# shravan-d/SculptMate

Measured on AMD Instinct MI355X. Metric: meshes/sec + ms/image, TripoSR 256^3 grid, at 1/2/4/8 MI355X, higher is better.
Workload: dtype fp32-equivalent (bf16 3-limb split, 24 bits, fp32 accumulate) density MLP / f32 tables, SiLU, marching cubes / bf16 transformer [filtered grid: an fp16 one-product pass decides the SIGN away from the level, every value marching cubes reads carries the three-limb value: mesh bit-identical to the full

## Files before the change

### include/sculpt_hip.h

```cpp
#ifndef SCULPT_HIP_H
#define SCULPT_HIP_H

#include <stddef.h>
#include <stdint.h>

#ifdef __cplusplus
extern "C" {
#endif

#define SCULPT_ABI_VERSION 4

typedef void *sculpt_stream_t;

int sculpt_version(void);
const char *sculpt_source_digest(void);
const char *sculpt_last_error(void);
int sculpt_device_count(void);
int sculpt_stream_create_cu_mask(int first_cu, int n_cus, sculpt_stream_t *stream_out);
int sculpt_stream_destroy(sculpt_stream_t stream);

size_t sculpt_mlp_packed_bytes(int in_channels, int n_hidden_64);
int sculpt_mlp_pack(const float *const *W_host, const float *const *b_host, int n_layers,
                    const int *dims_host, void *packed_host, size_t packed_bytes);

// ... 201 lines not shown
                         sculpt_stream_t stream);

int sculpt_resize_aa_bilinear(const float *in_hwc, int Hin, int Win, int C, float *tmp, float *out_hwc, int Hout,
                              int Wout, sculpt_stream_t stream);

int sculpt_resample_lanczos_ksize(int in_size, int out_size);
int sculpt_resample_lanczos_coeffs(int in_size, int out_size, int ksize, int32_t *bounds_host, int32_t *kk_host);
int sculpt_resample_u8(const uint8_t *in_hwc, int Hin, int Win, int C, const int32_t *bounds_x, const int32_t *kk_x, int ksize_x,
                       const int32_t *bounds_y, const int32_t *kk_y, int ksize_y, uint8_t *tmp, uint8_t *out_hwc, int Hout, int Wout,
                       sculpt_stream_t stream);
int sculpt_u2net_input(const uint8_t *img_hwc, int H, int W, int C, const double *mean3_host, const double *std3_host, int32_t *ws,
                       float *out_chw, sculpt_stream_t stream);
int sculpt_u2net_mask(const float *d0, int64_t n, uint32_t *ws, uint8_t *mask, sculpt_stream_t stream);
int sculpt_cutout_bbox(const uint8_t *img_hwc, const uint8_t *mask, int H, int W, int C, int32_t *ws, int32_t *bbox_host,
                       sculpt_stream_t stream);
int sculpt_cutout_frame(const uint8_t *img_hwc, const uint8_t *mask, int H, int W, int C, int y0, int x0, int h, int w, int top,
                        int left, int S, int grey, uint8_t *out, sculpt_stream_t stream);
int sculpt_u8_to_unit_f32(const uint8_t *in, int64_t n, float *out, sculpt_stream_t stream);

int sculpt_vit_patchify(const float *image_hwc, int S, int P, const float *mean3_host, const float *std3_host,
                        uint16_t *patches, float *patches_f32 , int ld, sculpt_stream_t stream);
int sculpt_vit_assemble(const float *patch_out, const float *cls, const float *pos, float *tokens,
                        int n_patches, int hidden, sculpt_stream_t stream);

int sculpt_upsample_scatter(const float *g, int ldg, const float *bias, float *planes, int S, int Co,
                            sculpt_stream_t stream);

size_t sculpt_bake_workspace_bytes(int res);
int sculpt_bake_rasterize(const float *uv, size_t nv, const int *idx, size_t nf, int res, void *workspace,
                          float *out, sculpt_stream_t stream);
int sculpt_bake_interpolate(const float *attr, size_t nv, const int *idx, size_t nf, const float *rast, int res,
                            float *out, sculpt_stream_t stream);
void rasterize_cpu(const float *uv, size_t nv, const int *idx, size_t nf, long long res, float *out);
void interpolate_cpu(const float *attr, size_t nv, const int *idx, size_t nf, const float *rast, long long res,
                     float *out);

int sculpt_im2col3x3(const void *in, int n_planes, int S, int C, int elem_bytes, void *out, sculpt_stream_t stream);
int sculpt_pixel_shuffle(const float *g, int ldg, float *planes, int n_planes, int S, int Co, int r,
                         sculpt_stream_t stream);

int sculpt_normalize_rows3(const float *x, int64_t n, float eps, float *y, sculpt_stream_t stream);

int sculpt_bake_material(const float *rast, int res, const float *color, const float *perturb_normal, const float *nrm,
                         const float *tng, float *albedo, float *bump, sculpt_stream_t stream);

int sculpt_uv_cell_atlas(const float *v_pos, const void *faces, int faces_i64, int64_t nf, int cols, int rows, float padding,
// ... 146 lines not shown
```

### sculptmate_amd/_lib.py

```python
import ctypes
import os

import torch

_HERE = os.path.dirname(os.path.abspath(__file__))
SO_PATH = os.path.join(_HERE, "libsculpt_hip.so")


class SculptError(RuntimeError):
    def __init__(self, msg, code=1):
        super().__init__(msg)
        self.code = code


if not os.path.exists(SO_PATH):
    raise ImportError(
        "sculptmate_amd: %s is missing -- build it with `python -m sculptmate_amd.build` "
        "(or __graft_entry__.build()); there is no CPU fallback." % SO_PATH)


def _load_matching_library():
    from . import build as _build

    if os.environ.get("SCULPT_ALLOW_STALE_LIB") == "1":
# ... 80 lines not shown
    "sculpt_maxpool2x2_ceil": (_i, [_vp, _i, _i, _i, _i, _vp, _i, _vp]),
    "sculpt_upsample_bilinear_bf16": (_i, [_vp, _i, _i, _i, _i, _vp, _i, _i, _i, _vp]),
    "sculpt_upsample_bilinear_f32": (_i, [_vp, _i, _i, _i, _vp, _i, _i, _vp]),
    "sculpt_add_bf16": (_i, [_vp, _i, _vp, _i, _vp, _i, _i64, _i, _vp]),
    "sculpt_fuse_sigmoid": (_i, [_vp, _i, _i64, _vp, _f, _vp, _vp]),
    "sculpt_gemm_f32": (_i, [_vp, _i, _vp, _i, _vp, _vp, _i, _vp, _i, _vp, _i, _i, _i, _i, _i, _i, _f, _i, _vp]),
    "sculpt_attention_f32_l3": (_i, [_vp, _i, _vp, _i, _vp, _i, _vp, _i, _i, _i, _i, _f, _vp]),
    "sculpt_limbs_bytes": (_sz, [_i, _i, _i]),
    "sculpt_attention_f32_l3_batched": (_i, [_vp, _i, _i64, _vp, _i, _i64, _vp, _i, _i64, _vp, _i, _i64, _vp, _i, _i, _i, _i, _i, _i, _i, _i, _f, _i, _vp]),
    "sculpt_layernorm_limbs": (_i, [_vp, _i, _vp, _vp, _f, _vp, _i, _vp, _i, _i, _i, _vp]),
    "sculpt_attention_f32_l3_limbs": (_i, [_vp, _i, _vp, _i, _vp, _i, _vp, _i, _i, _i, _i, _i, _i, _f, _i, _vp]),
    "sculpt_limbs_split": (_i, [_vp, _i, _i, _i, _f, _i, _vp, _vp]),
    "sculpt_gemm_l3p": (_i, [_vp, _vp, _i, _f, _vp, _vp, _i, _vp, _i, _vp, _i, _i, _vp, _i, _i, _i, _i, _i, _vp]),
    "sculpt_gemm_f32_ex": (_i, [_vp, _i, _vp, _i, _vp, _vp, _i, _vp, _i, _vp, _i, _i, _i, _i, _i, _i, _f, _i, _i, _i, _i64, _i64, _i64, _vp]),
    "sculpt_softmax_rows_f32": (_i, [_vp, _i, _i, _i, _i, _vp]),
    "sculpt_attention_bf16": (_i, [_vp, _i, _vp, _i, _vp, _i, _vp, _i, _i, _i, _i, _f, _vp]),
    "sculpt_attention_bf16_prescaled": (_i, [_vp, _i, _vp, _i, _vp, _i, _vp, _i, _i, _i, _i, _vp]),
    "sculpt_attention_bf16_batched": (_i, [_vp, _i, _i64, _vp, _i, _i64, _vp, _i, _i64, _vp, _i, _i64, _i, _i, _i, _i, _i, _f, _vp]),
    "sculpt_layernorm": (_i, [_vp, _vp, _i, _vp, _vp, _f, _vp, _i, _vp, _i, _i, _vp]),
    "sculpt_groupnorm_tokens": (_i, [_vp, _i, _i, _i, _vp, _vp, _f, _vp, _vp, _vp, _vp]),
    "sculpt_transpose_add": (_i, [_vp, _vp, _vp, _i, _i, _vp]),
    "sculpt_vit_patchify": (_i, [_vp, _i, _i, _vp, _vp, _vp, _vp, _i, _vp]),
    "sculpt_vit_assemble": (_i, [_vp, _vp, _vp, _vp, _i, _i, _vp]),
    "sculpt_upsample_scatter": (_i, [_vp, _i, _vp, _vp, _i, _i, _vp]),
    "sculpt_cast_bf16": (_i, [_vp, _vp, _i64, _vp]),
    "sculpt_dilate_fill": (_i, [_vp, _vp, _i, _i, _i, _vp, _vp, _vp]),
    "sculpt_vertex_accumulate_workspace_bytes": (_sz, [_sz]),
    "sculpt_vertex_normals": (_i, [_vp, _sz, _vp, _i, _sz, _vp, _vp, _vp]),
    "sculpt_vertex_tangents": (_i, [_vp, _vp, _vp, _sz, _vp, _i, _sz, _vp, _vp, _vp]),
    "sculpt_resize_aa_bilinear": (_i, [_vp, _i, _i, _i, _vp, _vp, _i, _i, _vp]),
    "sculpt_resample_lanczos_ksize": (_i, [_i, _i]),
    "sculpt_resample_lanczos_coeffs": (_i, [_i, _i, _i, _vp, _vp]),
    "sculpt_resample_u8": (_i, [_vp, _i, _i, _i, _vp, _vp, _i, _vp, _vp, _i, _vp, _vp, _i, _i, _vp]),
    "sculpt_u2net_input": (_i, [_vp, _i, _i, _i, _vp, _vp, _vp, _vp, _vp]),
    "sculpt_u2net_mask": (_i, [_vp, _i64, _vp, _vp, _vp]),
    "sculpt_cutout_bbox": (_i, [_vp, _vp, _i, _i, _i, _vp, _vp, _vp]),
    "sculpt_cutout_frame": (_i, [_vp, _vp, _i, _i, _i, _i, _i, _i, _i, _i, _i, _i, _i, _vp, _vp]),
    "sculpt_u8_to_unit_f32": (_i, [_vp, _i64, _vp, _vp]),
    "sculpt_bake_workspace_bytes": (_sz, [_i]),
    "sculpt_bake_rasterize": (_i, [_vp, _sz, _vp, _sz, _i, _vp, _vp, _vp]),
    "sculpt_bake_interpolate": (_i, [_vp, _sz, _vp, _sz, _vp, _i, _vp, _vp]),
    "sculpt_im2col3x3": (_i, [_vp, _i, _i, _i, _i, _vp, _vp]),
    "sculpt_pixel_shuffle": (_i, [_vp, _i, _vp, _i, _i, _i, _i, _vp]),
    "sculpt_uv_stats_words": (_sz, []),
    "sculpt_uv_moments_workspace_bytes": (_sz, []),
    "sculpt_uv_moments": (_i, [_vp, _sz, _vp, _vp, _vp]),
# ... 116 lines not shown
```

### sculptmate_amd/csrc/norms.hip

```cpp
#include "common.h"
#include "limbs.h"

namespace sculpt {

__device__ __forceinline__ float wave_sum(float v) {
#pragma unroll
    for (int d = 32; d >= 1; d >>= 1) v += __shfl_xor(v, d, 64);
    return v;
}

template <bool IN_BF16>
__global__ __launch_bounds__(256) void layernorm_kernel(const float *__restrict__ xf, const uint16_t *__restrict__ xb,
                                                        int ldx, const float *__restrict__ gamma,
                                                        const float *__restrict__ beta, float eps,
                                                        uint16_t *__restrict__ y, int ldy, float *__restrict__ yf,
                                                        int rows, int cols, unsigned char *__restrict__ y_lt = nullptr, int lt_fmt = 0) {
    const int lane = threadIdx.x & 63;
    const int row = blockIdx.x * 4 + (threadIdx.x >> 6);
    if (row >= rows) return;
    constexpr int MAXV = 8;
    float v[MAXV][4];
    const int nv = cols / 256;
    float s = 0.f;
#pragma unroll
// ... 158 lines not shown
    }
}

__global__ __launch_bounds__(256) void upsample_scatter_kernel(const float *__restrict__ g, int ldg,
                                                               const float *__restrict__ bias, float *__restrict__ planes,
                                                               int S, int Co) {
    const int S2 = 2 * S;
    const long total = 3L * Co * S2 * S2;
    for (long i = (long)blockIdx.x * 256 + threadIdx.x; i < total; i += (long)gridDim.x * 256) {
        const int X = (int)(i % S2), Y = (int)((i / S2) % S2);
        const int co = (int)((i / ((long)S2 * S2)) % Co), pl = (int)(i / ((long)S2 * S2 * Co));
        const int w = X >> 1, dx = X & 1, hh = Y >> 1, dy = Y & 1;
        const long tok = (long)pl * S * S + (long)hh * S + w;
        planes[i] = g[tok * ldg + co * 4 + dy * 2 + dx] + bias[co];
    }
}

__global__ __launch_bounds__(256) void cast_bf16_kernel(const float *__restrict__ x, uint16_t *__restrict__ y, long n) {
    for (long i = (long)blockIdx.x * 256 + threadIdx.x; i < n; i += (long)gridDim.x * 256) y[i] = f32_to_bf16(x[i]);
}

static inline int grid_for(long n) { return (int)std::min<long>((n + 255) / 256, 2048); }

__global__ __launch_bounds__(256) void row_slice_stats_kernel(const float *__restrict__ x, int ldx, int rows, int slots,
                                                              float *__restrict__ stats, int stats_ld,
                                                              uint16_t *__restrict__ xb, int ldb) {
    const long t = (long)blockIdx.x * 256 + threadIdx.x;
    if (t >= (long)rows * slots) return;
    const int slot = (int)(t / rows), row = (int)(t % rows);
    const float4 *src = reinterpret_cast<const float4 *>(x + (long)row * ldx + slot * 64);
    float4 v[16];
    float s = 0.f;
#pragma unroll
    for (int i = 0; i < 16; ++i) { v[i] = src[i]; s += (v[i].x + v[i].y) + (v[i].z + v[i].w); }
    const float mean = s * (1.0f / 64.0f);
    float m2 = 0.f;
#pragma unroll
    for (int i = 0; i < 16; ++i) {
        const float a = v[i].x - mean, b = v[i].y - mean, c = v[i].z - mean, d = v[i].w - mean;
        m2 = fmaf(a, a, m2); m2 = fmaf(b, b, m2); m2 = fmaf(c, c, m2); m2 = fmaf(d, d, m2);
    }
    reinterpret_cast<float2 *>(stats)[(long)slot * stats_ld + row] = make_float2(mean, m2);
    if (xb) {
        uint2 *dst = reinterpret_cast<uint2 *>(xb + (long)row * ldb + slot * 64);
#pragma unroll
        for (int i = 0; i < 16; ++i) {
            uint2 pk;
            pk.x = pack_bf16x2(v[i].x, v[i].y);
            pk.y = pack_bf16x2(v[i].z, v[i].w);
            dst[i] = pk;
        }
    }
}

}

using namespace sculpt;

extern "C" {

int sculpt_row_slice_stats(const float *x, int ldx, int rows, int cols, float *stats, int stats_ld, uint16_t *x_bf16, int ldb,
                           sculpt_stream_t stream) {
    SC_REQUIRE(x && stats && stats_ld >= rows, "row_slice_stats: null argument or stats_ld < rows");
    SC_REQUIRE(cols >= 64 && cols % 64 == 0 && ldx % 4 == 0 && (!x_bf16 || ldb % 4 == 0), "row_slice_stats: cols=%d must be a multiple of 64", cols);
    if (rows <= 0) return 0;
    const int slots = cols / 64;
    hipLaunchKernelGGL(row_slice_stats_kernel, dim3(cdiv((long)rows * slots, 256)), dim3(256), 0, as_stream(stream), x, ldx, rows,
                       slots, stats, stats_ld, x_bf16, ldb);
    SC_LAUNCH_CHECK();
    return 0;
}

int sculpt_layernorm(const float *x_f32, const uint16_t *x_bf16, int ldx, const float *gamma, const float *beta,
                     float eps, uint16_t *y, int ldy, float *y_f32, int rows, int cols, sculpt_stream_t stream) {
    SC_REQUIRE((x_f32 != nullptr) != (x_bf16 != nullptr), "layernorm: give exactly one of x_f32 / x_bf16");
// ... 51 lines not shown

int sculpt_vit_patchify(const float *image_hwc, int S, int P, const float *mean3_host, const float *std3_host,
                        uint16_t *patches, float *patches_f32, int ld, sculpt_stream_t stream) {
    SC_REQUIRE(image_hwc && mean3_host && std3_host && (patches || patches_f32), "vit_patchify: null argument");
    SC_REQUIRE(P > 0 && S >= P, "vit_patchify: bad S=%d P=%d", S, P);
    if (ld <= 0) ld = 3 * P * P;
    SC_REQUIRE(ld >= 3 * P * P, "vit_patchify: ld=%d < 3*P*P", ld);
    const long total = (long)(S / P) * (S / P) * ld;
    hipLaunchKernelGGL(patchify_kernel, dim3(grid_for(total)), dim3(256), 0, as_stream(stream), image_hwc, S, P, ld,
                       mean3_host[0], mean3_host[1], mean3_host[2], std3_host[0], std3_host[1], std3_host[2], patches, patches_f32);
    SC_LAUNCH_CHECK();
    return 0;
}

int sculpt_vit_assemble(const float *patch_out, const float *cls, const float *pos, float *tokens, int n_patches,
                        int hidden, sculpt_stream_t stream) {
    SC_REQUIRE(patch_out && cls && pos && tokens, "vit_assemble: null argument");
    hipLaunchKernelGGL(vit_assemble_kernel, dim3(grid_for((long)(n_patches + 1) * hidden)), dim3(256), 0,
                       as_stream(stream), patch_out, cls, pos, tokens, n_patches, hidden);
    SC_LAUNCH_CHECK();
    return 0;
}

int sculpt_upsample_scatter(const float *g, int ldg, const float *bias, float *planes, int S, int Co,
                            sculpt_stream_t stream) {
    SC_REQUIRE(g && bias && planes, "upsample_scatter: null argument");
    SC_REQUIRE(ldg >= 4 * Co, "upsample_scatter: ldg=%d < 4*Co", ldg);
    hipLaunchKernelGGL(upsample_scatter_kernel, dim3(grid_for(3L * Co * 4 * S * S)), dim3(256), 0, as_stream(stream), g,
                       ldg, bias, planes, S, Co);
    SC_LAUNCH_CHECK();
    return 0;
}

int sculpt_cast_bf16(const float *x, uint16_t *y, int64_t n, sculpt_stream_t stream) {
    SC_REQUIRE(x && y, "cast_bf16: null argument");
    if (n <= 0) return 0;
    hipLaunchKernelGGL(cast_bf16_kernel, dim3(grid_for(n)), dim3(256), 0, as_stream(stream), x, y, (long)n);
    SC_LAUNCH_CHECK();
    return 0;
}

}

namespace sculpt {

__device__ __forceinline__ void aa_taps(int i, int in_size, float scale, int *xmin, int *xsize, float *support_inv,
// ... 50 lines not shown
```

### sculptmate_amd/engine.py

```python
import os

import torch

from . import _lib, ops

BF16 = torch.bfloat16


def prepare_ln_linear(L, key, W, bias, gamma, beta, fold, to_weight, to_f32, q_rows=0, q_scale=1.0):
    W = torch.as_tensor(W)
    if fold:
        if q_rows:
            W = W.clone().to(torch.float32)
            W[:q_rows] *= q_scale
            if bias is not None:
                bias = torch.as_tensor(bias).clone().to(torch.float32)
                bias[:q_rows] *= q_scale
        Wp, bp, cs = ops.fold_layernorm(W, bias, gamma, beta)
        L[key], L[key + "_b"], L[key + "_cs"] = to_weight(Wp), to_f32(bp), to_f32(cs)
    else:
        L[key], L[key + "_b"] = to_weight(W), (None if bias is None else to_f32(bias))
        L[key + "_ln"] = (to_f32(gamma), to_f32(beta))


# ... 86 lines not shown
            st["xn"] = self._b(name + "_xn", (T, D), torch.float32)
        return st

    def _state_from(self, h, name="bb"):
        st = self._stream_state(name, h)
        self._stats_of(st)
        return st

    def _stats_of(self, st):
        if self.precision == "bf16":
            ops.row_slice_stats(st["h"], st["stats"], st["hb"])

    def _ln_gemm(self, st, L, key, eps, **kw):
        if self.precision == "bf16":
            return ops.gemm(st["hb"], L[key], bias=L[key + "_b"], ln_stats=st["stats"], ln_colsum=L[key + "_cs"], ln_eps=eps, **kw)
        g, b = L[key + "_ln"]
        if isinstance(L[key], ops.Limbs):
            xn = self._lt(st["name"] + "_xn", st["h"].shape[0], st["h"].shape[1])
            ops.layernorm(st["h"], g, b, eps, y_lt=xn)
            return self._gemm(xn, L[key], bias=L[key + "_b"], **kw)
        ops.layernorm(st["h"], g, b, eps, y_f32=st["xn"])
        return self._gemm(st["xn"], L[key], bias=L[key + "_b"], **kw)

    def _res_gemm(self, st, A, W, bias):
        h = st["h"]
        if self.precision == "bf16":
            return ops.gemm(A, W, bias=bias, residual=h, out_f32=h, out_bf16=st["hb"], stats_out=st["stats"])
        return self._gemm(A, W, bias=bias, residual=h, out_f32=h)
```

### sculptmate_amd/ops.py

```python
import ctypes
import math
import numbers
import threading
import os

import numpy as np
import torch

from . import _lib
from ._lib import SculptError, check, lib


def _stream():
    return ctypes.c_void_p(torch.cuda.current_stream().cuda_stream)


def _ptr(t):
    return ctypes.c_void_p(t.data_ptr()) if t is not None else ctypes.c_void_p(0)


def _req(t, dtype, name):
    if not (isinstance(t, torch.Tensor) and t.is_cuda):
        raise SculptError("%s must be a CUDA/HIP tensor (no CPU fallback)" % name)
    if t.dtype != dtype:
# ... 702 lines not shown
                                      _ptr(stats_ws), _stream()))


def transpose_add(x_tc, residual_ct, out_ct):
    T, C = x_tc.shape
    check(lib.sculpt_transpose_add(_ptr(x_tc), _ptr(residual_ct), _ptr(out_ct), T, C, _stream()))


def vit_patchify(image_hwc, patch, mean, std, patches):
    S = image_hwc.shape[0]
    m = (ctypes.c_float * 3)(*[float(v) for v in mean])
    s = (ctypes.c_float * 3)(*[float(v) for v in std])
    pb = patches if patches.dtype == BF16 else None
    pf = patches if patches.dtype == torch.float32 else None
    check(lib.sculpt_vit_patchify(_ptr(image_hwc), S, patch, ctypes.cast(m, ctypes.c_void_p),
                                  ctypes.cast(s, ctypes.c_void_p), _ptr(pb), _ptr(pf), patches.stride(0), _stream()))


def vit_assemble(patch_out, cls, pos, tokens):
    n_patches, hidden = patch_out.shape[0], patch_out.shape[1]
    check(lib.sculpt_vit_assemble(_ptr(patch_out), _ptr(cls), _ptr(pos), _ptr(tokens), n_patches, hidden, _stream()))


def upsample_scatter(g, bias, planes, S, Co):
    check(lib.sculpt_upsample_scatter(_ptr(g), g.stride(0), _ptr(bias), _ptr(planes), S, Co, _stream()))


def cast_bf16(x, y):
    check(lib.sculpt_cast_bf16(_ptr(x), _ptr(y), x.numel(), _stream()))


def bake_rasterize(uv, face_indices, bake_resolution):
    uv = _req(uv.contiguous(), torch.float32, "uv")
    idx = _req(face_indices.to(torch.int32).contiguous(), torch.int32, "face_indices")
    res = int(bake_resolution)
    ws = _workspace(("bake", uv.device), lib.sculpt_bake_workspace_bytes(res), uv.device)
    out = torch.empty((res, res, 4), dtype=torch.float32, device=uv.device)
    check(lib.sculpt_bake_rasterize(_ptr(uv), uv.shape[0], _ptr(idx), idx.shape[0], res, _ptr(ws), _ptr(out), _stream()))
    return out


def bake_interpolate(attr, rast, face_indices):
    attr = _req(attr.contiguous(), torch.float32, "attr")
    rast = _req(rast.contiguous(), torch.float32, "rast")
    idx = _req(face_indices.to(torch.int32).contiguous(), torch.int32, "face_indices")
    res = rast.shape[0]
# ... 486 lines not shown
```

### sculptmate_amd/tsr/system.py

```python
import math
import os
from typing import List, Optional

import numpy as np
import torch

from .. import _lib, ops
from ..engine import KernelEngine, prepare_ln_linear
from .posemb import interpolate_pos_embedding
from .cameras import get_spherical_cameras
from .utils import ImagePreprocessor

BF16 = torch.bfloat16
LOG2E = 1.4426950408889634

from .spec import DEFAULT_CFG, IMAGE_MEAN, IMAGE_STD, param_spec


class Mesh:

    def __init__(self, vertices, faces, vertex_colors=None, uvs=None, texture=None, vertex_normals=None):
        self.vertices = vertices
        self.faces = faces
        self.vertex_colors = vertex_colors
# ... 224 lines not shown
        self.decoder_filter = bool(decoder_filter)
        self.filter_info = {"margin": None, "coarse": "fp16", "usable": True, "calibrations": 0, "filtered": 0, "fallbacks": 0,
                            "last": None}
        self.cfg = cfg or DEFAULT_CFG
        self.pos_embed_mode = pos_embed_mode
        self.precision = precision
        self.l3p = False
        self.range_fallbacks = 0
        self._range_twin = None
        self.adt = BF16 if precision == "bf16" else torch.float32
        self._spec = param_spec(self.cfg)
        self._sd = None
        self.device = None
        self.renderer = TriplaneNeRFRenderer(self.cfg["renderer"])
        self.image_processor = ImagePreprocessor()
        self.isosurface_helper = None
        self.decoder = None
        self.mesh_sink = None
        self.textured_mesh_sink = None
        self._unwrapper = None
        self.max_batch = 1
        self.batch_exact = True
        self._w = None
        self._pos_cache = {}
        self._buf = {}

    @classmethod
    def from_pretrained(cls, pretrained_model_name_or_path: str, config_name: str, weight_name: str, **model_kwargs):
        if not os.path.isdir(pretrained_model_name_or_path):
            raise FileNotFoundError("Checkpoint directory given doesnt exist")
        cfg = load_config(os.path.join(pretrained_model_name_or_path, config_name),
                          os.path.join(pretrained_model_name_or_path, "config.json"))
        model = cls(cfg, **model_kwargs)
        ckpt = torch.load(os.path.join(pretrained_model_name_or_path, weight_name), map_location="cpu")
        model.load_state_dict(ckpt)
        return model

    def state_dict(self):
        return dict(self._sd or {})

    def load_state_dict(self, sd, strict=True):
        sd = {k: (torch.from_numpy(np.ascontiguousarray(v)) if isinstance(v, np.ndarray) else v) for k, v in sd.items()}
        missing = [k for k in self._spec if k not in sd]
        unexpected = [k for k in sd if k not in self._spec]
        if strict and (missing or unexpected):
            raise RuntimeError("Error(s) in loading state_dict for TSR: missing %s unexpected %s"
# ... 86 lines not shown
            L["sa_o"], L["sa_ob"] = wh(sd[q + "attn1.to_out.0.weight"], dev), _f32(sd[q + "attn1.to_out.0.bias"], dev)
            ln_linear(L, "ca_q", sd[q + "attn2.to_q.weight"], None, sd[q + "norm2.weight"], sd[q + "norm2.bias"], q_rows=Db, q_scale=qs)
            L["_ca_k"], L["_ca_v"] = sd[q + "attn2.to_k.weight"], sd[q + "attn2.to_v.weight"]
            L["ca_o"], L["ca_ob"] = wh(sd[q + "attn2.to_out.0.weight"], dev), _f32(sd[q + "attn2.to_out.0.bias"], dev)
            ln_linear(L, "ff1", sd[q + "ff.net.0.proj.weight"], sd[q + "ff.net.0.proj.bias"], sd[q + "norm3.weight"], sd[q + "norm3.bias"],
                      geglu=True)
            L["ff2"], L["ff2_b"] = wh(sd[q + "ff.net.2.weight"], dev), _f32(sd[q + "ff.net.2.bias"], dev)
            w["blocks"].append(L)
        w["ca_kv_all"] = wh(torch.cat([L.pop("_ca_k") for L in w["blocks"]] + [L.pop("_ca_v") for L in w["blocks"]], 0), dev)
        up = sd["post_processor.upsample.weight"]
        Co = up.shape[1]
        rows = up.permute(1, 2, 3, 0).reshape(4 * Co, up.shape[0])
        npad = ((4 * Co + 127) // 128) * 128
        upw = torch.zeros(npad, up.shape[0])
        upw[: 4 * Co] = rows
        w["up_w"], w["up_b"] = wt(upw, dev), _f32(sd["post_processor.upsample.bias"], dev)
        self._w = w
        d = cfg["decoder"]
        n = d["n_hidden_layers"] + 1
        self.decoder = ops.PackedMLP([sd["decoder.layers.%d.weight" % (2 * i)] for i in range(n)],
                                     [sd["decoder.layers.%d.bias" % (2 * i)] for i in range(n)], dev)
        self._pos_cache = {}
        self._buf = {}

    def _pos(self, n_side, dev):
        if n_side not in self._pos_cache:
            pe = self._sd["image_tokenizer.model.embeddings.position_embeddings"].numpy()
            self._pos_cache[n_side] = _f32(interpolate_pos_embedding(pe, n_side, self.pos_embed_mode), dev)
        return self._pos_cache[n_side]

    @staticmethod
    def _token_stride(T, B):
        return T if B == 1 else ((T + 7) // 8) * 8

    def image_tokens(self, image_hwc):
        imgs = list(image_hwc) if isinstance(image_hwc, (list, tuple)) else [image_hwc]
        B = len(imgs)
        v, w = self.cfg["image_tokenizer"], self._w
        H, P, nh = v["hidden_size"], v["patch_size"], v["num_attention_heads"]
        S = imgs[0].shape[0]
        if any(tuple(im.shape) != tuple(imgs[0].shape) for im in imgs):
            raise ValueError("TSR.image_tokens: the images of a batch must have one size")
        n_side = S // P
        npatch = n_side * n_side
        T = npatch + 1
        Ts = self._token_stride(T, B)
        M = B * Ts
        ldt = ((((B - 1) * Ts + ((T + 63) // 64) * 64) + 63) // 64) * 64
        patches = self._b("patches", (B * npatch, 3 * P * P), self.adt)
        for b, im in enumerate(imgs):
            ops.vit_patchify(im, P, IMAGE_MEAN, IMAGE_STD, patches[b * npatch:(b + 1) * npatch])
        pout = self._b("patch_out", (B * npatch, H), torch.float32)
        self._gemm(patches, w["patch_w"], bias=w["patch_b"], out_f32=pout)
        h = self._b("vit_h", (M, H), torch.float32, zero=True)
        pos = self._pos(n_side, imgs[0].device)
        for b in range(B):
            ops.vit_assemble(pout[b * npatch:(b + 1) * npatch], w["cls"], pos, h[b * Ts:b * Ts + T])
            if Ts > T:
                h[b * Ts + T:(b + 1) * Ts].zero_()
        st = self._stream_state("vit", h)
        self._stats_of(st)
        qk = self._b("vit_qk", (M, 2 * H), self.adt)
        vt = self._b("vit_vt", (H, ldt), self.adt, zero=True)
        if self.l3p:
            att, ff = self._lt("vit_att", M, H), self._lt("vit_ff", M, v["intermediate_size"])
        else:
            att = self._b("vit_att", (M, H), self.adt, zero=True)
            ff = self._b("vit_ff", (M, v["intermediate_size"]), self.adt)
        eps = v["layer_norm_eps"]
        for L in w["vit"]:
            self._ln_gemm(st, L, "qkv_w", eps, out_bf16=qk, out_t=vt, n_split=2 * H)
            self._attn(qk[:, :H], qk[:, H:], vt, att, T, T, nh, self._attn_scale(1.0 / math.sqrt(H // nh)),
                       B, Ts * 2 * H, Ts * 2 * H, Ts, Ts * H)
            self._res_gemm(st, att, L["o_w"], L["o_b"])
            self._ln_gemm(st, L, "f1_w", eps, out_bf16=ff, epilogue=_lib.EPI_GELU)
            self._res_gemm(st, ff, L["f2_w"], L["f2_b"])
        ctx32 = self._b("ctx32", (M, H), torch.float32)
        if self.precision == "bf16":
            ctx = self._b("ctx", (M, H), BF16)
            ops.layernorm(h, w["vit_ln_w"], w["vit_ln_b"], eps, y=ctx, y_f32=ctx32)
        elif self.l3p:
            ctx = self._lt("ctx", M, H)
            ops.layernorm(h, w["vit_ln_w"], w["vit_ln_b"], eps, y_lt=ctx, y_f32=ctx32)
        else:
            ops.layernorm(h, w["vit_ln_w"], w["vit_ln_b"], eps, y_f32=ctx32)
            ctx = ctx32
        return ctx, ctx32

    def _attn_scale(self, scale):
        return None if self.precision == "bf16" else scale

    def _self_attention(self, st, L, batch=1):
        b = self.cfg["backbone"]
        nh, hd = b["num_attention_heads"], b["attention_head_dim"]
        D, M = nh * hd, st["h"].shape[0]
        T = M // batch
        Mp = ((((batch - 1) * T + ((T + 63) // 64) * 64) + 63) // 64) * 64
        qk = self._b("bb_qk", (M, 2 * D), self.adt)
        vt = self._b("bb_vt", (D, Mp), self.adt, zero=True)
        att = self._lt("bb_att", M, D) if self.l3p else self._b("bb_att", (M, D), self.adt)
        self._ln_gemm(st, L, "sa_qkv", 1e-5, out_bf16=qk, out_t=vt, n_split=2 * D)
        self._attn(qk[:, :D], qk[:, D:], vt, att, T, T, nh, self._attn_scale(1.0 / math.sqrt(hd)),
                   batch, T * 2 * D, T * 2 * D, T, T * D)
        self._res_gemm(st, att, L["sa_o"], L["sa_ob"])

    def _run_blocks(self, st, ctx: torch.Tensor, first_self_attention_done: bool = False, batch: int = 1, ctx_tokens=None):
        b, w = self.cfg["backbone"], self._w
        nh, hd = b["num_attention_heads"], b["attention_head_dim"]
        D = nh * hd
        if self.l3p and not isinstance(ctx, ops.Limbs):
            ctx = ops.Limbs.of(ctx.to(torch.float32).contiguous(), fmt=self.limb_format)
        M, Mc = st["h"].shape[0], (ctx.rows if isinstance(ctx, ops.Limbs) else ctx.shape[0])
        T, Ts = M // batch, Mc // batch
        Tc = Ts if ctx_tokens is None else ctx_tokens
        ldc = ((((batch - 1) * Ts + ((Tc + 63) // 64) * 64) + 63) // 64) * 64
        q = self._b("bb_q", (M, D), self.adt)
        nL = len(w["blocks"])
        ck_all = self._b("bb_ck", (Mc, nL * D), self.adt)
        cvt_all = self._b("bb_cvt", (nL * D, ldc), self.adt, zero=True)
        self._gemm(ctx, w["ca_kv_all"], out_bf16=ck_all, out_t=cvt_all, n_split=nL * D, M=Mc)
        if self.l3p:
            att, ff = self._lt("bb_att", M, D), self._lt("bb_ff", M, 4 * D)
        else:
            att = self._b("bb_att", (M, D), self.adt)
            ff = self._b("bb_ff", (M, 4 * D), self.adt)
        scale = self._attn_scale(1.0 / math.sqrt(hd))
        for li, L in enumerate(w["blocks"]):
            ck, cvt = ck_all[:, li * D:(li + 1) * D], cvt_all[li * D:(li + 1) * D]
            if li > 0 or not first_self_attention_done:
                self._self_attention(st, L, batch)
            self._ln_gemm(st, L, "ca_q", 1e-5, out_bf16=q)
            self._attn(q, ck, cvt, att, T, Tc, nh, scale, batch, T * D, Ts * nL * D, Ts, T * D)
            self._res_gemm(st, att, L["ca_o"], L["ca_ob"])
            self._ln_gemm(st, L, "ff1", 1e-5, out_bf16=ff, epilogue=_lib.EPI_GEGLU)
            self._res_gemm(st, ff, L["ff2"], L["ff2_b"])
        return st

    def _backbone_head(self):
        b, w = self.cfg["backbone"], self._w
        D = b["num_attention_heads"] * b["attention_head_dim"]
        T = w["emb_ct"].shape[1]
        xn = self._b("bb_xn", (T, w["emb_ct"].shape[0]), self.adt)
        stats = self._b("gn_stats", (2 * b["norm_num_groups"],), torch.float32)
        ops.groupnorm_tokens(w["emb_ct"], b["norm_num_groups"], w["gn_w"], w["gn_b"], 1e-6, xn, stats)
        h = self._b("bb_h", (T, D), torch.float32)
        st = self._stream_state("bb", h)
        if self.precision == "bf16":
            ops.gemm(xn, w["pin_w"], bias=w["pin_b"], out_f32=h, out_bf16=st["hb"], stats_out=st["stats"])
        else:
            self._gemm(xn, w["pin_w"], bias=w["pin_b"], out_f32=h)
        return st

    def _backbone_tail(self, st, batch=1):
        w = self._w
        C = self.cfg["tokenizer"]["num_channels"]
        h = st["h"]
        M, D = h.shape
        res = w["emb_tc"]
        if batch > 1:
            key = "emb_tc_x%d" % batch
            if key not in w:
                w[key] = res.repeat(batch, 1).contiguous()
            res = w[key]
        out = self._b("bb_out", (M, C), torch.float32)
        if self.precision == "bf16":
            outb = self._b("bb_outb", (M, C), BF16)
            ops.gemm(st["hb"], w["pout_w"], bias=w["pout_b"], residual=res, out_f32=out, out_bf16=outb)
        else:
            ops.gemm_f32(h, w["pout_w"], bias=w["pout_b"], residual=res, out=out, l3=self.l3)
            outb = out
        return out, outb

    def _broadcast_state(self, st1, batch):
        T, D = st1["h"].shape
        st = self._stream_state("bb", self._b("bb_h", (batch * T, D), torch.float32))
        st["h"].view(batch, T, D).copy_(st1["h"][None])
        if self.precision == "bf16":
            st["hb"].view(batch, T, D).copy_(st1["hb"][None])
            st["stats"].view(-1, batch, T, 2).copy_(st1["stats"][:, None])
        return st

    def encode_images(self, images):
        B = len(images)
        if B == 1:
            return self.encode_image(images[0])
        main = torch.cuda.current_stream(self.device)
        last_tok = getattr(self, "_tok_last", None)
        if last_tok is not None:
            main.wait_event(last_tok)
        side = getattr(self, "_side_stream", None)
        if side is None:
            side = self._side_stream = torch.cuda.Stream(self.device)
        fork, join = torch.cuda.Event(), torch.cuda.Event()
        fork.record(main)
        with torch.cuda.stream(side):
            side.wait_event(fork)
            st1 = self._backbone_head()
            self._self_attention(st1, self._w["blocks"][0])
            st = self._broadcast_state(st1, B)
            join.record(side)
        T = self.cfg["image_tokenizer"]
        n_side = images[0].shape[0] // T["patch_size"]
        with ops.single_image_tiles(n_side * n_side + 1 if self.batch_exact else 0):
            ctx, _ = self.image_tokens(list(images))
        main.wait_event(join)
        with ops.single_image_tiles(3 * self.cfg["tokenizer"]["plane_size"] ** 2 if self.batch_exact else 0):
            st = self._run_blocks(st, ctx, first_self_attention_done=True, batch=B, ctx_tokens=n_side * n_side + 1)
            return self._backbone_tail(st, B)

    def backbone_tokens(self, ctx: torch.Tensor):
        st = self._run_blocks(self._backbone_head(), ctx)
        return self._backbone_tail(st)

    def encode_image(self, image_hwc: torch.Tensor):
        main = torch.cuda.current_stream(self.device)
        last_tok = getattr(self, "_tok_last", None)
        if last_tok is not None:
            main.wait_event(last_tok)
        side = getattr(self, "_side_stream", None)
        if side is None:
            side = self._side_stream = torch.cuda.Stream(self.device)
        fork, join = torch.cuda.Event(), torch.cuda.Event()
        fork.record(main)
        with torch.cuda.stream(side):
            side.wait_event(fork)
            st = self._backbone_head()
            self._self_attention(st, self._w["blocks"][0])
            join.record(side)
        ctx, _ = self.image_tokens(image_hwc)
        main.wait_event(join)
        st = self._run_blocks(st, ctx, first_self_attention_done=True)
        return self._backbone_tail(st)

    def _preprocess(self, im) -> torch.Tensor:
        size = self.cfg["cond_image_size"]
        img = self._upload(_to_float_hwc(im)).contiguous()
        if img.shape[-1] != 3:
            raise ValueError("TSR.forward expects RGB images (composite RGBA on grey first, preprocessing.py:122)")
        if img.shape[0] != size or img.shape[1] != size:
            img = ops.resize_aa_bilinear(img, size)
        return img

    def tokens_async(self, image) -> PendingTokens:
        if self._w is None:
            raise _lib.SculptError("TSR: call load_state_dict() and to(device) before tokens_async()")
        tok = getattr(self, "_tok_stream", None)
        if tok is None:
            tok = self._tok_stream = torch.cuda.Stream(self.device)
            self._tok_ring = {"i": 0, "slots": [{"ctx": None, "consumed": None} for _ in range(2)]}
        slot = self._tok_ring["slots"][self._tok_ring["i"] % 2]
        self._tok_ring["i"] += 1
        main = torch.cuda.current_stream(self.device)
        fork = torch.cuda.Event()
        fork.record(main)
        with torch.cuda.stream(tok), torch.no_grad():
            tok.wait_event(fork)
            if slot["consumed"] is not None:
                tok.wait_event(slot["consumed"])
            ctx, _ = self.image_tokens(self._preprocess(image))
            if isinstance(ctx, ops.Limbs):
                if not isinstance(slot["ctx"], ops.Limbs) or (slot["ctx"].rows, slot["ctx"].cols, slot["ctx"].fmt) != (ctx.rows, ctx.cols, ctx.fmt):
                    slot["ctx"] = ops.Limbs(ctx.rows, ctx.cols, data=torch.empty_like(ctx.data), fmt=ctx.fmt)
                slot["ctx"].data.copy_(ctx.data)
            else:
                if not isinstance(slot["ctx"], torch.Tensor) or slot["ctx"].shape != ctx.shape or slot["ctx"].dtype != ctx.dtype:
                    slot["ctx"] = torch.empty_like(ctx)
                slot["ctx"].copy_(ctx)
            ready = torch.cuda.Event()
            ready.record(tok)
        self._tok_last = ready
        return PendingTokens(slot["ctx"], ready, slot, image)

    def forward_tokens(self, tokens: PendingTokens) -> torch.Tensor:
        main = torch.cuda.current_stream(self.device)
        main.wait_event(tokens.ready)
        st = self._run_blocks(self._backbone_head(), tokens.ctx)
        consumed = torch.cuda.Event()
        consumed.record(main)
        tokens._slot["consumed"] = consumed
        _, outb = self._backbone_tail(st)
        out = self.scene_code(outb)[None]
        if self.precision == "fp16l2" and tokens.image is not None and not bool(torch.isfinite(out).all()):
            return self._range_fallback([tokens.image])
        return out

    def scene_code(self, tokens_bf16: torch.Tensor, batch: int = 1):
        w = self._w
        S = self.cfg["tokenizer"]["plane_size"]
        Co = self.cfg["post_processor"]["out_channels"]
        g = self._b("up_g", (tokens_bf16.shape[0], w["up_w"].shape[0]), torch.float32)
        self._gemm(tokens_bf16, w["up_w"], out_f32=g)
        planes = torch.empty((batch, 3, Co, 2 * S, 2 * S), dtype=torch.float32, device=tokens_bf16.device)
        T = tokens_bf16.shape[0] // batch
        for b in range(batch):
            ops.upsample_scatter(g[b * T:(b + 1) * T], w["up_b"], planes[b], S, Co)
        return planes if batch > 1 else planes[0]

    def _upload(self, t: torch.Tensor) -> torch.Tensor:
        if t.device.type != "cpu":
# ... 469 lines not shown
```

Measured before the change: 118.3.

## Cache image-independent backbone head and fuse ViT assemble with row stats

The backbone head (learned triplane tokens, first self-attention and first cross-attention query projection) does not depend on the input image, so it is now computed once per weight/precision configuration, cached, and reused for every image instead of being recomputed on a side stream. The first block then starts directly from the cached query and residual. Separately, the ViT token assembly (cls + patch + pos add) is fused with the per-slice mean/M2 statistics and bf16 copy for the single-image bf16 path, which removes a separate stats pass. The cache adds memory and a one-time synchronize, and relies on the head being truly input-independent.

```diff
diff --git a/include/sculpt_hip.h b/include/sculpt_hip.h
--- a/include/sculpt_hip.h
+++ b/include/sculpt_hip.h
@@ -247,6 +247,8 @@
                         uint16_t *patches, float *patches_f32 , int ld, sculpt_stream_t stream);
 int sculpt_vit_assemble(const float *patch_out, const float *cls, const float *pos, float *tokens,
                         int n_patches, int hidden, sculpt_stream_t stream);
+int sculpt_vit_assemble_stats(const float *patch_out, const float *cls, const float *pos, float *tokens, int ldt, int n_patches,
+                              int hidden, float *stats, int stats_ld, uint16_t *tokens_bf16, int ldb, sculpt_stream_t stream);
 
 int sculpt_upsample_scatter(const float *g, int ldg, const float *bias, float *planes, int S, int Co,
                             sculpt_stream_t stream);
diff --git a/sculptmate_amd/_lib.py b/sculptmate_amd/_lib.py
--- a/sculptmate_amd/_lib.py
+++ b/sculptmate_amd/_lib.py
@@ -126,6 +126,7 @@
     "sculpt_transpose_add": (_i, [_vp, _vp, _vp, _i, _i, _vp]),
     "sculpt_vit_patchify": (_i, [_vp, _i, _i, _vp, _vp, _vp, _vp, _i, _vp]),
     "sculpt_vit_assemble": (_i, [_vp, _vp, _vp, _vp, _i, _i, _vp]),
+    "sculpt_vit_assemble_stats": (_i, [_vp, _vp, _vp, _vp, _i, _i, _i, _vp, _i, _vp, _i, _vp]),
     "sculpt_upsample_scatter": (_i, [_vp, _i, _vp, _vp, _i, _i, _vp]),
     "sculpt_cast_bf16": (_i, [_vp, _vp, _i64, _vp]),
     "sculpt_dilate_fill": (_i, [_vp, _vp, _i, _i, _i, _vp, _vp, _vp]),
diff --git a/sculptmate_amd/csrc/norms.hip b/sculptmate_amd/csrc/norms.hip
--- a/sculptmate_amd/csrc/norms.hip
+++ b/sculptmate_amd/csrc/norms.hip
@@ -204,6 +204,31 @@
 
 static inline int grid_for(long n) { return (int)std::min<long>((n + 255) / 256, 2048); }
 
+__device__ __forceinline__ void slice_stats_store(const float4 (&v)[16], int row, int slot, float *__restrict__ stats, int stats_ld,
+                                                  uint16_t *__restrict__ xb, int ldb) {
+    float s = 0.f;
+#pragma unroll
+    for (int i = 0; i < 16; ++i) s += (v[i].x + v[i].y) + (v[i].z + v[i].w);
+    const float mean = s * (1.0f / 64.0f);
+    float m2 = 0.f;
+#pragma unroll
+    for (int i = 0; i < 16; ++i) {
+        const float a = v[i].x - mean, b = v[i].y - mean, c = v[i].z - mean, d = v[i].w - mean;
+        m2 = fmaf(a, a, m2); m2 = fmaf(b, b, m2); m2 = fmaf(c, c, m2); m2 = fmaf(d, d, m2);
+    }
+    reinterpret_cast<float2 *>(stats)[(long)slot * stats_ld + row] = make_float2(mean, m2);
+    if (xb) {
+        uint2 *dst = reinterpret_cast<uint2 *>(xb + (long)row * ldb + slot * 64);
+#pragma unroll
+        for (int i = 0; i < 16; ++i) {
+            uint2 pk;
+            pk.x = pack_bf16x2(v[i].x, v[i].y);
+            pk.y = pack_bf16x2(v[i].z, v[i].w);
+            dst[i] = pk;
+        }
+    }
+}
+
 __global__ __launch_bounds__(256) void row_slice_stats_kernel(const float *__restrict__ x, int ldx, int rows, int slots,
                                                               float *__restrict__ stats, int stats_ld,
                                                               uint16_t *__restrict__ xb, int ldb) {
@@ -212,27 +237,30 @@
     const int slot = (int)(t / rows), row = (int)(t % rows);
     const float4 *src = reinterpret_cast<const float4 *>(x + (long)row * ldx + slot * 64);
     float4 v[16];
-    float s = 0.f;
-#pragma unroll
-    for (int i = 0; i < 16; ++i) { v[i] = src[i]; s += (v[i].x + v[i].y) + (v[i].z + v[i].w); }
-    const float mean = s * (1.0f / 64.0f);
-    float m2 = 0.f;
+#pragma unroll
+    for (int i = 0; i < 16; ++i) v[i] = src[i];
+    slice_stats_store(v, row, slot, stats, stats_ld, xb, ldb);
+}
+
+__global__ __launch_bounds__(256) void vit_assemble_stats_kernel(const float *__restrict__ patch_out, const float *__restrict__ cls,
+                                                                 const float *__restrict__ pos, float *__restrict__ tokens, int ldt,
+                                                                 int rows, int slots, float *__restrict__ stats, int stats_ld,
+                                                                 uint16_t *__restrict__ xb, int ldb) {
+    const long t = (long)blockIdx.x * 256 + threadIdx.x;
+    if (t >= (long)rows * slots) return;
+    const int slot = (int)(t / rows), row = (int)(t % rows);
+    const int hidden = slots * 64;
+    const float4 *src = reinterpret_cast<const float4 *>((row == 0 ? cls : patch_out + (long)(row - 1) * hidden) + slot * 64);
+    const float4 *ps = reinterpret_cast<const float4 *>(pos + (long)row * hidden + slot * 64);
+    float4 *dst = reinterpret_cast<float4 *>(tokens + (long)row * ldt + slot * 64);
+    float4 v[16];
 #pragma unroll
     for (int i = 0; i < 16; ++i) {
-        const float a = v[i].x - mean, b = v[i].y - mean, c = v[i].z - mean, d = v[i].w - mean;
-        m2 = fmaf(a, a, m2); m2 = fmaf(b, b, m2); m2 = fmaf(c, c, m2); m2 = fmaf(d, d, m2);
-    }
-    reinterpret_cast<float2 *>(stats)[(long)slot * stats_ld + row] = make_float2(mean, m2);
-    if (xb) {
-        uint2 *dst = reinterpret_cast<uint2 *>(xb + (long)row * ldb + slot * 64);
-#pragma unroll
-        for (int i = 0; i < 16; ++i) {
-            uint2 pk;
-            pk.x = pack_bf16x2(v[i].x, v[i].y);
-            pk.y = pack_bf16x2(v[i].z, v[i].w);
-            dst[i] = pk;
-        }
-    }
+        const float4 a = src[i], p = ps[i];
+        v[i] = make_float4(a.x + p.x, a.y + p.y, a.z + p.z, a.w + p.w);
+        dst[i] = v[i];
+    }
+    slice_stats_store(v, row, slot, stats, stats_ld, xb, ldb);
 }
 
 }
@@ -330,6 +358,21 @@
     return 0;
 }
 
+int sculpt_vit_assemble_stats(const float *patch_out, const float *cls, const float *pos, float *tokens, int ldt, int n_patches,
+                              int hidden, float *stats, int stats_ld, uint16_t *tokens_bf16, int ldb, sculpt_stream_t stream) {
+    SC_REQUIRE(patch_out && cls && pos && tokens && stats, "vit_assemble_stats: null argument");
+    SC_REQUIRE(n_patches >= 0 && stats_ld >= n_patches + 1, "vit_assemble_stats: stats_ld=%d < %d rows", stats_ld, n_patches + 1);
+    SC_REQUIRE(hidden >= 64 && hidden % 64 == 0 && ldt >= hidden && ldt % 4 == 0 && (!tokens_bf16 || (ldb >= hidden && ldb % 4 == 0)),
+               "vit_assemble_stats: hidden=%d must be a multiple of 64, ldt / ldb multiples of 4 and >= hidden", hidden);
+    SC_REQUIRE((((uintptr_t)patch_out | (uintptr_t)cls | (uintptr_t)pos | (uintptr_t)tokens) & 15) == 0 && ((uintptr_t)tokens_bf16 & 7) == 0 &&
+               ((uintptr_t)stats & 7) == 0, "vit_assemble_stats: arrays must be 16-byte aligned");
+    const int rows = n_patches + 1, slots = hidden / 64;
+    hipLaunchKernelGGL(vit_assemble_stats_kernel, dim3(cdiv((long)rows * slots, 256)), dim3(256), 0, as_stream(stream), patch_out, cls,
+                       pos, tokens, ldt, rows, slots, stats, stats_ld, tokens_bf16, ldb);
+    SC_LAUNCH_CHECK();
+    return 0;
+}
+
 int sculpt_upsample_scatter(const float *g, int ldg, const float *bias, float *planes, int S, int Co,
                             sculpt_stream_t stream) {
     SC_REQUIRE(g && bias && planes, "upsample_scatter: null argument");
diff --git a/sculptmate_amd/engine.py b/sculptmate_amd/engine.py
--- a/sculptmate_amd/engine.py
+++ b/sculptmate_amd/engine.py
@@ -132,8 +132,9 @@
         ops.layernorm(st["h"], g, b, eps, y_f32=st["xn"])
         return self._gemm(st["xn"], L[key], bias=L[key + "_b"], **kw)
 
-    def _res_gemm(self, st, A, W, bias):
+    def _res_gemm(self, st, A, W, bias, residual=None):
         h = st["h"]
+        res = h if residual is None else residual
         if self.precision == "bf16":
-            return ops.gemm(A, W, bias=bias, residual=h, out_f32=h, out_bf16=st["hb"], stats_out=st["stats"])
-        return self._gemm(A, W, bias=bias, residual=h, out_f32=h)
+            return ops.gemm(A, W, bias=bias, residual=res, out_f32=h, out_bf16=st["hb"], stats_out=st["stats"])
+        return self._gemm(A, W, bias=bias, residual=res, out_f32=h)
diff --git a/sculptmate_amd/ops.py b/sculptmate_amd/ops.py
--- a/sculptmate_amd/ops.py
+++ b/sculptmate_amd/ops.py
@@ -748,6 +748,13 @@
     check(lib.sculpt_vit_assemble(_ptr(patch_out), _ptr(cls), _ptr(pos), _ptr(tokens), n_patches, hidden, _stream()))
 
 
+def vit_assemble_stats(patch_out, cls, pos, tokens, stats, tokens_bf16=None):
+    n_patches, hidden = patch_out.shape[0], patch_out.shape[1]
+    check(lib.sculpt_vit_assemble_stats(_ptr(patch_out), _ptr(cls), _ptr(pos), _ptr(tokens), tokens.stride(0), n_patches, hidden,
+                                        _ptr(stats), stats.shape[1], _ptr(tokens_bf16),
+                                        tokens_bf16.stride(0) if tokens_bf16 is not None else 0, _stream()))
+
+
 def upsample_scatter(g, bias, planes, S, Co):
     check(lib.sculpt_upsample_scatter(_ptr(g), g.stride(0), _ptr(bias), _ptr(planes), S, Co, _stream()))
 
diff --git a/sculptmate_amd/tsr/system.py b/sculptmate_amd/tsr/system.py
--- a/sculptmate_amd/tsr/system.py
+++ b/sculptmate_amd/tsr/system.py
@@ -270,6 +270,7 @@
         self.max_batch = 1
         self.batch_exact = True
         self._w = None
+        self._head0 = None
         self._pos_cache = {}
         self._buf = {}
 
@@ -402,6 +403,7 @@
                                      [sd["decoder.layers.%d.bias" % (2 * i)] for i in range(n)], dev)
         self._pos_cache = {}
         self._buf = {}
+        self._head0 = None
 
     def _pos(self, n_side, dev):
         if n_side not in self._pos_cache:
@@ -434,12 +436,15 @@
         self._gemm(patches, w["patch_w"], bias=w["patch_b"], out_f32=pout)
         h = self._b("vit_h", (M, H), torch.float32, zero=True)
         pos = self._pos(n_side, imgs[0].device)
-        for b in range(B):
-            ops.vit_assemble(pout[b * npatch:(b + 1) * npatch], w["cls"], pos, h[b * Ts:b * Ts + T])
-            if Ts > T:
-                h[b * Ts + T:(b + 1) * Ts].zero_()
         st = self._stream_state("vit", h)
-        self._stats_of(st)
+        if B == 1 and self.precision == "bf16":
+            ops.vit_assemble_stats(pout, w["cls"], pos, h, st["stats"], st["hb"])
+        else:
+            for b in range(B):
+                ops.vit_assemble(pout[b * npatch:(b + 1) * npatch], w["cls"], pos, h[b * Ts:b * Ts + T])
+                if Ts > T:
+                    h[b * Ts + T:(b + 1) * Ts].zero_()
+            self._stats_of(st)
         qk = self._b("vit_qk", (M, 2 * H), self.adt)
         vt = self._b("vit_vt", (H, ldt), self.adt, zero=True)
         if self.l3p:
@@ -484,7 +489,7 @@
                    batch, T * 2 * D, T * 2 * D, T, T * D)
         self._res_gemm(st, att, L["sa_o"], L["sa_ob"])
 
-    def _run_blocks(self, st, ctx: torch.Tensor, first_self_attention_done: bool = False, batch: int = 1, ctx_tokens=None):
+    def _run_blocks(self, st, ctx: torch.Tensor, first_self_attention_done: bool = False, batch: int = 1, ctx_tokens=None, head=None):
         b, w = self.cfg["backbone"], self._w
         nh, hd = b["num_attention_heads"], b["attention_head_dim"]
         D = nh * hd
@@ -507,11 +512,20 @@
         scale = self._attn_scale(1.0 / math.sqrt(hd))
         for li, L in enumerate(w["blocks"]):
             ck, cvt = ck_all[:, li * D:(li + 1) * D], cvt_all[li * D:(li + 1) * D]
-            if li > 0 or not first_self_attention_done:
-                self._self_attention(st, L, batch)
-            self._ln_gemm(st, L, "ca_q", 1e-5, out_bf16=q)
-            self._attn(q, ck, cvt, att, T, Tc, nh, scale, batch, T * D, Ts * nL * D, Ts, T * D)
-            self._res_gemm(st, att, L["ca_o"], L["ca_ob"])
+            if li == 0 and head is not None:
+                if batch == 1:
+                    self._attn(head["q0"], ck, cvt, att, T, Tc, nh, scale)
+                    self._res_gemm(st, att, L["ca_o"], L["ca_ob"], residual=head["h0"])
+                else:
+                    q.view(batch, T, D).copy_(head["q0"][None])
+                    self._attn(q, ck, cvt, att, T, Tc, nh, scale, batch, T * D, Ts * nL * D, Ts, T * D)
+                    self._res_gemm(st, att, L["ca_o"], L["ca_ob"])
+            else:
+                if li > 0 or not first_self_attention_done:
+                    self._self_attention(st, L, batch)
+                self._ln_gemm(st, L, "ca_q", 1e-5, out_bf16=q)
+                self._attn(q, ck, cvt, att, T, Tc, nh, scale, batch, T * D, Ts * nL * D, Ts, T * D)
+                self._res_gemm(st, att, L["ca_o"], L["ca_ob"])
             self._ln_gemm(st, L, "ff1", 1e-5, out_bf16=ff, epilogue=_lib.EPI_GEGLU)
             self._res_gemm(st, ff, L["ff2"], L["ff2_b"])
         return st
@@ -530,6 +544,27 @@
         else:
             self._gemm(xn, w["pin_w"], bias=w["pin_b"], out_f32=h)
         return st
+
+    def _backbone_head_cached(self):
+        key = (self.precision, self.limb_format, self.l3p)
+        hc = self._head0
+        if hc is not None and hc["key"] == key:
+            return hc
+        with ops.single_image_tiles(0):
+            st = self._backbone_head()
+            L = self._w["blocks"][0]
+            self._self_attention(st, L)
+            q = self._b("bb_q", st["h"].shape, self.adt)
+            self._ln_gemm(st, L, "ca_q", 1e-5, out_bf16=q)
+        hc = {"key": key, "h0": st["h"].clone(), "q0": q.clone()}
+        if self.precision == "bf16":
+            hc["hb0"], hc["stats0"] = st["hb"].clone(), st["stats"].clone()
+        torch.cuda.current_stream(self.device).synchronize()
+        self._head0 = hc
+        return hc
+
+    def _head_state(self, hc):
+        return self._stream_state("bb", self._b("bb_h", tuple(hc["h0"].shape), torch.float32))
 
     def _backbone_tail(self, st, batch=1):
         w = self._w
@@ -551,13 +586,13 @@
             outb = out
         return out, outb
 
-    def _broadcast_state(self, st1, batch):
-        T, D = st1["h"].shape
+    def _broadcast_state(self, hc, batch):
+        T, D = hc["h0"].shape
         st = self._stream_state("bb", self._b("bb_h", (batch * T, D), torch.float32))
-        st["h"].view(batch, T, D).copy_(st1["h"][None])
+        st["h"].view(batch, T, D).copy_(hc["h0"][None])
         if self.precision == "bf16":
-            st["hb"].view(batch, T, D).copy_(st1["hb"][None])
-            st["stats"].view(-1, batch, T, 2).copy_(st1["stats"][:, None])
+            st["hb"].view(batch, T, D).copy_(hc["hb0"][None])
+            st["stats"].view(-1, batch, T, 2).copy_(hc["stats0"][:, None])
         return st
 
     def encode_images(self, images):
@@ -568,28 +603,19 @@
         last_tok = getattr(self, "_tok_last", None)
         if last_tok is not None:
             main.wait_event(last_tok)
-        side = getattr(self, "_side_stream", None)
-        if side is None:
-            side = self._side_stream = torch.cuda.Stream(self.device)
-        fork, join = torch.cuda.Event(), torch.cuda.Event()
-        fork.record(main)
-        with torch.cuda.stream(side):
-            side.wait_event(fork)
-            st1 = self._backbone_head()
-            self._self_attention(st1, self._w["blocks"][0])
-            st = self._broadcast_state(st1, B)
-            join.record(side)
+        hc = self._backbone_head_cached()
         T = self.cfg["image_tokenizer"]
         n_side = images[0].shape[0] // T["patch_size"]
         with ops.single_image_tiles(n_side * n_side + 1 if self.batch_exact else 0):
             ctx, _ = self.image_tokens(list(images))
-        main.wait_event(join)
+        st = self._broadcast_state(hc, B)
         with ops.single_image_tiles(3 * self.cfg["tokenizer"]["plane_size"] ** 2 if self.batch_exact else 0):
-            st = self._run_blocks(st, ctx, first_self_attention_done=True, batch=B, ctx_tokens=n_side * n_side + 1)
+            st = self._run_blocks(st, ctx, batch=B, ctx_tokens=n_side * n_side + 1, head=hc)
             return self._backbone_tail(st, B)
 
     def backbone_tokens(self, ctx: torch.Tensor):
-        st = self._run_blocks(self._backbone_head(), ctx)
+        hc = self._backbone_head_cached()
+        st = self._run_blocks(self._head_state(hc), ctx, head=hc)
         return self._backbone_tail(st)
 
     def encode_image(self, image_hwc: torch.Tensor):
@@ -597,19 +623,9 @@
         last_tok = getattr(self, "_tok_last", None)
         if last_tok is not None:
             main.wait_event(last_tok)
-        side = getattr(self, "_side_stream", None)
-        if side is None:
-            side = self._side_stream = torch.cuda.Stream(self.device)
-        fork, join = torch.cuda.Event(), torch.cuda.Event()
-        fork.record(main)
-        with torch.cuda.stream(side):
-            side.wait_event(fork)
-            st = self._backbone_head()
-            self._self_attention(st, self._w["blocks"][0])
-            join.record(side)
+        hc = self._backbone_head_cached()
         ctx, _ = self.image_tokens(image_hwc)
-        main.wait_event(join)
-        st = self._run_blocks(st, ctx, first_self_attention_done=True)
+        st = self._run_blocks(self._head_state(hc), ctx, head=hc)
         return self._backbone_tail(st)
 
     def _preprocess(self, im) -> torch.Tensor:
@@ -654,7 +670,8 @@
     def forward_tokens(self, tokens: PendingTokens) -> torch.Tensor:
         main = torch.cuda.current_stream(self.device)
         main.wait_event(tokens.ready)
-        st = self._run_blocks(self._backbone_head(), tokens.ctx)
+        hc = self._backbone_head_cached()
+        st = self._run_blocks(self._head_state(hc), tokens.ctx, head=hc)
         consumed = torch.cuda.Event()
         consumed.record(main)
         tokens._slot["consumed"] = consumed
```

New measurement: 120.1, median of 6. +1.5%, better.
